# fmfi-compbio/nadavca

Measured on AMD Instinct MI355X. Metric: reads/sec (align_signal, ~4k-sample reads), higher is better.
Workload: dtype f64

## Files before the change

### nadavca_amd/csrc/api.hip

```cpp
#include <math.h>
#include <stdarg.h>
#include <stdio.h>
#include <stdlib.h>
#include <string.h>

#include <new>
#include <vector>

#include "nvk_internal.h"

static thread_local char g_err[512] = "";

void nvk_set_error(const char *fmt, ...) {
  va_list ap;
  va_start(ap, fmt);
  vsnprintf(g_err, sizeof g_err, fmt, ap);
  va_end(ap);
}

extern "C" const char *nvk_last_error(void) { return g_err; }

extern "C" int nvk_device_count(void) {
  int n = 0;
  if (hipGetDeviceCount(&n) != hipSuccess) return 0;
// ... 387 lines not shown
  }
  NVK_HIP(hipSetDevice(model->ctx->device));
  a = BatchArgs{n_reads, total_signal, total_ref, total_anchors, signal, sig_off, reference, ref_off,
                ctx_before, cb_off, ctx_after, ca_off, anchors, anc_off, bandwidth, mel};
  return NVK_OK;
}

struct PlanHost {
  PlanTotals tot;
  int32_t steps[1];
};

int plan_batch_queue(nvk_model *model, const BatchArgs &a, int mode, int write_rows, const int **order,
                     const std::function<int()> *meanwhile) {
  nvk_ctx *ctx = model->ctx;
  int64_t n = a.n_reads;
  int64_t rows_total = (mode == PLAN_ALIGN_TRANS) ? 2 * a.total_ref : a.total_ref + n;
  int rc;
  ctx->rows_current = 0;
  if ((rc = nvk_ws_reserve(ctx, WS_META, (size_t)(n + 1) * sizeof(ReadMeta) + 64))) return rc;
  if ((rc = nvk_ws_reserve(ctx, WS_ROWS, (size_t)(rows_total + 1) * sizeof(RowParam)))) return rc;
  if ((rc = nvk_ws_reserve(ctx, WS_BANDTMP, (size_t)(2 * (a.total_ref + n) + 2) * 8))) return rc;
  if ((rc = nvk_ws_reserve(ctx, WS_MISC, 256))) return rc;
  if ((rc = nvk_ws_reserve(ctx, WS_LANE_F, (size_t)(rows_total + 1) * 48))) return rc;
  if ((rc = nvk_ws_reserve(ctx, WS_LANE_R, (size_t)(rows_total + 1) * 48))) return rc;
  if ((rc = nvk_ws_reserve(ctx, WS_OFFS, (size_t)(rows_total + 1) * sizeof(int32_t)))) return rc;
  if ((rc = nvk_ws_reserve(ctx, WS_STEPS, (size_t)(n + 1) * sizeof(int32_t)))) return rc;
  if ((rc = nvk_ws_reserve(ctx, WS_ORDER, (size_t)n * sizeof(int) + 4096))) return rc;
  if ((rc = nvk_grow(&ctx->h_plan, &ctx->h_plan_cap, sizeof(PlanHost) + (size_t)n * sizeof(int32_t), true,
                     "planner results")))
    return rc;
  PlanTotals *d_tot = nvk_plan_totals(ctx);
  rc = launch_plan(ctx, model->dm, a, mode, (ReadMeta *)ctx->ws[WS_META],
                   (RowParam *)ctx->ws[WS_ROWS], (unsigned long long *)ctx->ws[WS_BANDTMP], d_tot,
                   ctx->ws[WS_LANE_F], ctx->ws[WS_LANE_R], (int32_t *)ctx->ws[WS_OFFS], write_rows, meanwhile);
  if (rc) return rc;
  ctx->rows_current = write_rows ? 1 : 0;
  int *ord = nullptr;
  rc = launch_order(ctx, (const ReadMeta *)ctx->ws[WS_META], n, d_tot, &ord, (int32_t *)ctx->ws[WS_STEPS]);
  if (rc) return rc;
  *order = ord;
  return NVK_OK;
}

int plan_batch_wait(nvk_ctx *ctx, int64_t n, PlanTotals &tot, const int32_t **steps_sorted) {
  PlanHost *hp = (PlanHost *)ctx->h_plan;
  NVK_HIP(hipMemcpyAsync(&hp->tot, nvk_plan_totals(ctx), sizeof(PlanTotals), hipMemcpyDeviceToHost, ctx->stream));
  if (n) NVK_HIP(hipMemcpyAsync(hp->steps, ctx->ws[WS_STEPS], (size_t)n * sizeof(int32_t), hipMemcpyDeviceToHost,
// ... 299 lines not shown
```

### nadavca_amd/csrc/kernels_align.hip

```cpp
#include <math.h>

#include "nvk_internal.h"
#include "wave.h"
#include "xmath.h"

namespace {

using xm::X;

constexpr int CH = 128;
constexpr int TABN = 128;
constexpr int PF = 4;

struct AlignArgs {
  const ReadMeta *metas;
  const RowParam *rows;
  const double *signal;
  double *spill_m;
  int32_t *spill_e;
  uint32_t *bp;
  int64_t spill_stride;
  int64_t bp_stride;
  int n_reads;
  int *counter;
// ... 327 lines not shown
            e = density(ring[(i - 1) & RM], mean, ac2, mc2);
            su = (su + 1 == H) ? 0 : su + 1;
            sA = (sA + 1 == H) ? 0 : sA + 1;
            sB = (sB + 1 == H) ? 0 : sB + 1;
            WAVE_SYNC();
          }
        }
#pragma unroll
        for (int q = 0; q < PF; q++) {
          cur_m[q] = nxt_m[q];
          cur_e[q] = nxt_e[q];
        }
      }
    }
    __syncthreads();

    int idx = __shfl(fidx, top & 63, 64);
    if (idx < 0) {
      if (lane == 0) g.out_status[rd] = NVK_READ_NO_PATH;
      continue;
    }
    {
      const bool ax = __any(amb_x), an = __any(amb_n), au = __any(amb_u);
      if ((ax || an || au || m.rsv) && lane == 0)
        g.ties[rd] = (ax ? NVK_TIE_EXACT : 0) | (an ? NVK_TIE_NEAR : 0) | (au ? NVK_TIE_ULP : 0) |
                     (m.rsv ? NVK_TIE_PLATEAU : 0);
    }
    if (lane == 0) {
      int32_t *ev = g.out_events + 2 * m.ref_off;
      int st = NVK_READ_OK;
      for (int r = top; r >= 0; --r) {
        if (g.transitions) {
          ev[2 * (r >> 1) + (r & 1)] = idx;
        } else {
          if (r > 0) ev[2 * (r - 1) + 1] = idx;
          if (r < top) ev[2 * r] = idx;
        }
        if (r == 0) break;
        const int pm = g.transitions ? ((r - 1) & 1 ? 0 : MEL) : MEL;
        int u = idx + c * r - t_min;
        int w = u >> 5;
        uint32_t v = bp[(size_t)w * 64 + (r & 63)] & (0xffffffffu >> (31 - (u & 31)));
        while (v == 0 && w > 0) {
          --w;
          v = bp[(size_t)w * 64 + (r & 63)];
        }
        if (v == 0) {
          st = NVK_READ_NO_PATH;
          break;
// ... 120 lines not shown
```

### nadavca_amd/csrc/kernels_align3.hip

```cpp
#include <math.h>

#include <new>
#include <vector>

#include "nvk_internal.h"
#include "xmath.h"
#include "dens.h"
#include "lane3.h"
#include "wave.h"

namespace {

using dens::density;
using dens::density_begin;
using dens::density_end;
using dens::DensHalf;
using dens::ETN;

constexpr int CH = 64;
static_assert(CH == 64, "a refill is one sample per lane");
constexpr int PF = 8;
constexpr int RU = 16;
constexpr int FT = 16;
static_assert(FT % PF == 0 && 32 % FT == 0, "forward trip");
// ... 9 lines not shown
typedef int v4i_t __attribute__((ext_vector_type(4)));
__device__ __forceinline__ void spill_store2(__amdgpu_buffer_rsrc_t rs, int lane16, int pair, double v_even,
                                             double v_odd) {
  __builtin_amdgcn_raw_buffer_store_b128(__builtin_bit_cast(v4i_t, make_double2(v_even, v_odd)), rs, lane16,
                                         pair * 1024, SPILL_AUX);
}
__device__ __forceinline__ double2 spill_load2(__amdgpu_buffer_rsrc_t rs, int lane16, int pair) {
  return __builtin_bit_cast(double2, __builtin_amdgcn_raw_buffer_load_b128(rs, lane16, pair * 1024, SPILL_AUX));
}

#define STEP_SYNC()                                                              \
  do {                                                                           \
    if (W == 1) WAVE_SYNC();                                                     \
    else asm volatile("s_waitcnt lgkmcnt(0)\n\ts_barrier" ::: "memory");         \
  } while (0)
#define RING_SYNC()                 \
  do {                              \
    if (W == 1) __syncthreads();    \
    else WAVE_SYNC();               \
  } while (0)

struct Align3Args {
  const ReadMeta *metas;
  const Lane3 *fwdl;
  const Lane3 *revl;
  const int32_t *offs;
  const double *signal;
  double *spill_v;
  int32_t *spill_L;
  uint32_t *bp;
  int64_t spill_stride;
  int64_t L_stride;
  int64_t bp_stride;
  int n_reads;
  int *counter;
  const int *order;
  int H, SR;
  int transitions;
  int c_cap;
  int flag_above;
  int2 *rstate;
  int read_lo;
  int *n_retry;
  int32_t *ties;
  int32_t *out_events;
  int32_t *out_status;
};

#define TAKE_LANE(l)                                                                   \
  do {                                                                                 \
    if (!PAIR || em) { mean = (l).mean; ac2 = (l).ac; mc2 = (l).mc; }   \
    melr = (l).mg & 15;                                                                \
    D = ((l).mg >> 4) & 255;                                                           \
    bs = (l).bs; pA = (l).pA; pW = (l).pW;                                             \
    ra = (int)min((unsigned)(su - D), (unsigned)(su - D + H)) * TL + nb;               \
    if (!PAIR) { pm = melr ? 1.0 : 0.0; qm = melr ? 0.0 : 1.0; }                       \
    if (PAIR && !em) cq = (shift_now != 0) ? ldexp((l).mean, shift_now) : (l).mean;    \
  } while (0)

__device__ __forceinline__ Lane3 lane3_sload(const Lane3 *p) {
  typedef const __attribute__((address_space(4))) v4i_t *cptr_t;
  cptr_t q = (cptr_t)(uintptr_t)p;
  const v4i_t q0 = q[0], q1 = q[1], q2 = q[2];
  Lane3 l;
  l.mean = __hiloint2double(q0.y, q0.x);
  l.ac = __hiloint2double(q0.w, q0.z);
  l.mc = __hiloint2double(q1.y, q1.x);
  l.bs = q1.z; l.end = q1.w;
  l.lo = q2.x; l.pA = q2.y; l.pW = q2.z; l.mg = q2.w;
  return l;
}

__device__ __forceinline__ int pair_swap(int v) { return __builtin_amdgcn_mov_dpp(v, 0xB1, 0xf, 0xf, true); }
__device__ __forceinline__ double pair_swap(double v) {
  return __hiloint2double(pair_swap(__double2hiint(v)), pair_swap(__double2loint(v)));
}

template <int MEL>
__device__ __forceinline__ double emission_product(double e, double e1, double e2, double e3) {
  double P = 1.0;
  if (MEL >= 1) P = e;
  if (MEL >= 2) P = P * e1;
  if (MEL >= 3) P = P * e2;
  if (MEL >= 4) P = P * e3;
  return P;
}

__device__ __forceinline__ int wave_max_i(int v) {
  for (int d = 32; d >= 1; d >>= 1) v = max(v, __shfl_xor(v, d, 64));
  return __builtin_amdgcn_readfirstlane(v);
}

struct Scale {
// ... 37 lines not shown
    }
  }
  unsigned char *histb = reinterpret_cast<unsigned char *>(hist2);
  unsigned char *ghistb = reinterpret_cast<unsigned char *>(ghist);
  int gl16 = gl * 16, gl8 = gl * 8, HZv = HZ, HZ2v = (PHASE == 1) ? HZ : 2 * HZ;
  asm volatile("" : "+v"(gl16), "+v"(gl8), "+v"(HZv), "+v"(HZ2v));
  const int lane16 = (W == 1) ? gl16 : lane * 16;

  while (true) {
    __syncthreads();
    if (gl == 0) *s_read = atomicAdd(g.counter, 1);
    __syncthreads();
    const int pos0 = __builtin_amdgcn_readfirstlane(*s_read);
    if (pos0 >= g.n_reads) break;
    const int pos = pos0 + g.read_lo;
    const int rd = g.order ? g.order[pos] : pos;
    const ReadMeta m = g.metas[rd];
    if (m.status != NVK_READ_OK) {
      if (PHASE == 2 && gl == 0) g.out_status[rd] = m.status;
      continue;
    }
    if ((W > 1) != (m.cw != 0)) continue;
    const int cm = (W > 1) ? m.cw : m.c;
    if (cm > g.c_cap) {
      if (PHASE == 2 && g.flag_above && gl == 0) {
        g.out_status[rd] = NVK_READ_RETRY_INTERNAL;
        atomicAdd(g.n_retry, 1);
      }
      continue;
    }
    const size_t slot = (size_t)pos0;
    const __amdgpu_buffer_rsrc_t spill_rs = __builtin_amdgcn_make_buffer_rsrc(
        g.spill_v + (slot * W + wv) * g.spill_stride, 0, 0x7ffffff0, 0x00020000);
    int32_t *spill_L = g.spill_L + slot * g.L_stride;
    const int T = __builtin_amdgcn_readfirstlane(m.T);
    const int N = __builtin_amdgcn_readfirstlane(m.N);
    const int c = __builtin_amdgcn_readfirstlane(cm);
    const int t_min = __builtin_amdgcn_readfirstlane(m.t_min);
    const int n_steps = __builtin_amdgcn_readfirstlane(m.pad);
    const int t_max = t_min + n_steps - 1;
    const Lane3 *fwdl = g.fwdl + m.row_off;
    const Lane3 *revl = g.revl + m.row_off;
    const int32_t *offs = g.offs + m.row_off;
    const double *sig = g.signal + m.sig_off;
    const int top = T - 1;
    int K = 0;
    bool suspect = false;

    if (PHASE == 1) {
      int r = top - ((top - gl) & (TL - 1));
      double mean = 0, ac2 = 0, mc2 = 0;
      int bs = -0x40000000, hi = -0x40000000, pA = 0x40000000, pW = 0, melr = 0, D = 1;
      double pm = 0.0, qm = 1.0;
      const bool em = PAIR ? ((lane & 1) == 0) : true;
      double cq = 0.0;
      int ia = 0;
      int dsel = 0;
      int shift_now = 0;
      if (PAIR) { pm = em ? 1.0 : 0.0; qm = em ? 0.0 : 1.0; }
      int su = 0;
      const int nb = (gl + 1) & (TL - 1);
      int ra = (H - 1) * TL + nb;
      bool is_init = false;
      int i = t_max;
      if (r >= 0) {
        const Lane3 cu = revl[r];
        TAKE_LANE(cu);
        hi = cu.end;
        is_init = (r == top);
        i = t_max - offs[r];
      }
      double prev = 0.0, e1 = 1.0, e2 = 1.0, e3 = 1.0;
      double o_hold = 0.0;
      int kmax = -0x40000000;
      int r_old = (W == 1) ? top : max(wave_max_i(r), -1);
      int i_old = (r_old >= 0) ? __builtin_amdgcn_readlane(i, r_old & 63) : 0x40000000;
      int filled_lo = (i_old / CH + 1) * CH;
      while (i_old - 3 < filled_lo) {
        filled_lo -= CH;
        for (int q = lane; q < CH; q += 64) {
          int idx = filled_lo + q;
          ring[idx & RM] = (idx >= 0 && idx < N) ? sig[idx] : 0.0;
        }
      }
      double nxt;
      {
        const int idx = filled_lo - CH + lane;
        nxt = (idx >= 0 && idx < N) ? sig[idx] : 0.0;
      }
// ... 16 lines not shown
      for (int ub = 0; ub < n_steps; ub += RU) {
#pragma unroll
      for (int uq = 0; uq < RU; uq++) {
        const int u = ub + uq;
        const int t = t_max - u;
        const int age = u & (RS - 1);
        if (age == 0 && u > 0) {
          sc.L += sc.d_next;
          sc.d_last = sc.d_next;
          sh_until = (sc.d_next != 0) ? u + c + MEL : 0;
          sc.d_next = 0;
          if (PAIR) { cq = ldexp(cq, sc.d_last); dsel = 0; }
        }
        if (PAIR && age == 1 && u > 1) cq = ldexp(cq, -sc.d_last);
        shift_now = (age == 0 && u > 0) ? sc.d_last : 0;
        bool fin = (i < bs);
        if (__any(fin)) {
          bool redo = false;
          for (unsigned long long fm = __builtin_amdgcn_ballot_w64(fin); fm != 0; fm &= fm - 1) {
            const int fl = __builtin_ctzll(fm);
            const int rn = __builtin_amdgcn_readlane(r, fl) - TL;
            Lane3 nx;
            nx.mean = nx.ac = nx.mc = 0.0; nx.bs = nx.end = nx.lo = nx.pA = nx.pW = nx.mg = 0;
            if (rn >= 0) nx = lane3_sload(revl + rn);
            if (lane == fl) {
              r = rn;
              i += nx.mg >> 12;
              prev = 0.0;
              if (r >= 0) {
                TAKE_LANE(nx);
                hi = nx.end;
                is_init = false;
                redo = true;
              } else {
                hi = -0x40000000; bs = -0x40000000; pA = 0x40000000; pW = 0;
                if (PAIR && !em) cq = 0.0;
              }
            }
          }
          if (PAIR) {
            if (__any(redo && em)) {
              const double pmn = pair_swap(mean), pac = pair_swap(ac2), pmc = pair_swap(mc2);
              const int ip = pair_swap(i);
              if (!em) { mean = pmn; ac2 = pac; mc2 = pmc; }
              const int odd = u & 1;
              if (W > 1) {
                redo = em ? redo : !odd;
// ... 118 lines not shown
      suspect = (rs.y != 0);
    }
    __syncthreads();
    __builtin_amdgcn_s_dcache_inv();

    double fbest = 0.0, fthr = 0.0;
    int fidx = -1, fG = 0;
    unsigned long long amb_x = 0, amb_u = 0, amb_n = 0;
    {
      int r = gl;
      double mean = 0, ac2 = 0, mc2 = 0;
      int bs = 0, be = 0x40000000, lo = 0x40000000, pA = 0x40000000, pW = 0, melr = 0, D = 1;
      double pm = 0.0, qm = 1.0;
      const bool em = PAIR ? ((lane & 1) != 0) : true;
      double cq = 0.0;
      int ia = 0, dsel = 0, shift_now = 0;
      if (PAIR) { pm = em ? 1.0 : 0.0; qm = em ? 0.0 : 1.0; }
      int su = 0;
      const int nb = (gl - 1) & (TL - 1);
      int ra = (H - 1) * TL + nb;
      bool is_init = false;
      int i = t_min - 64 * c;
      if (r < T) {
        const Lane3 cu = fwdl[r];
        TAKE_LANE(cu);
        be = cu.end; lo = cu.lo;
        is_init = (r == 0);
        i = t_min - offs[r];
      }
      double prev = 0.0, e1 = 1.0, e2 = 1.0, e3 = 1.0;
      double bestn = 0.0, bthr = 0.0;
      int G = GBIG;
      double rsum = 0.0, smin = INFINITY, smax = 0.0;
      uint32_t bits = 0;
      int r_old = min(64 * wv, T);
      int i_old = (r_old < T) ? __builtin_amdgcn_readfirstlane(i) : -0x40000000;
      int filled_hi = ((i_old - MEL - 1) > 0 ? (i_old - MEL - 1) / CH : 0) * CH;
      while (i_old + 2 >= filled_hi) {
        for (int w = lane; w < CH; w += 64) {
          int idx = filled_hi + w;
          ring[idx & RM] = (idx >= 0 && idx < N) ? sig[idx] : 0.0;
        }
        filled_hi += CH;
      }
      double nxt;
      {
        const int idx = filled_hi + lane;
// ... 25 lines not shown
      for (int ub = 0; ub < n_steps; ub += FT) {
#pragma unroll
        for (int q = 0; q < FT; q++) {
          const int u = ub + q;
          {
            const int age = u & (RS - 1);
            if (age == 0 && u > 0) {
              sc.L += sc.d_next;
              sc.d_last = sc.d_next;
              sh_until = (sc.d_next != 0) ? u + c + MEL : 0;
              sc.d_next = 0;
              if (PAIR) { cq = ldexp(cq, sc.d_last); dsel = 0; }
            }
            if (PAIR && age == 1 && u > 1) cq = ldexp(cq, -sc.d_last);
            shift_now = (age == 0 && u > 0) ? sc.d_last : 0;
            bool fin = (i > be);
            if (__any(fin)) {
              bool redo = false;
              for (unsigned long long fm = __builtin_amdgcn_ballot_w64(fin); fm != 0; fm &= fm - 1) {
                const int fl = __builtin_ctzll(fm);
                const int rn = __builtin_amdgcn_readlane(r, fl) + TL;
                Lane3 nx;
                nx.mean = nx.ac = nx.mc = 0.0; nx.bs = nx.end = nx.lo = nx.pA = nx.pW = nx.mg = 0;
                if (rn < T) nx = lane3_sload(fwdl + rn);
                if (lane == fl) {
                  smin = fmin(smin, rsum);
                  smax = fmax(smax, rsum);
                  rsum = 0.0;
                  r = rn;
                  i -= nx.mg >> 12;
                  prev = 0.0;
                  bestn = 0.0; bthr = 0.0; G = GBIG;
                  if (r < T) {
                    TAKE_LANE(nx);
                    be = nx.end; lo = nx.lo;
                    is_init = false;
                    redo = true;
                  } else {
                    lo = 0x40000000; be = 0x40000000; pA = 0x40000000; pW = 0;
                    if (PAIR && !em) cq = 0.0;
                  }
                }
              }
              if (PAIR) {
                if (__any(redo && em)) {
                  const double pmn = pair_swap(mean), pac = pair_swap(ac2), pmc = pair_swap(mc2);
                  const int ip = pair_swap(i);
// ... 169 lines not shown
      if (lane == 0) tflag[wv] = (any_suspect ? 1 : 0) | (amb_x != 0 ? 2 : 0) | (amb_n != 0 ? 4 : 0) | (amb_u != 0 ? 8 : 0);
      if (gl == (top & (TL - 1))) *tfidx = fidx;
      __syncthreads();
      int fl = 0;
#pragma unroll
      for (int w = 0; w < W; w++) fl |= tflag[w];
      any_suspect = (fl & 1) != 0;
      amb_x = (fl & 2) ? 1ull : 0ull;
      amb_n = (fl & 4) ? 1ull : 0ull;
      amb_u = (fl & 8) ? 1ull : 0ull;
      idx = *tfidx;
    }
    if (any_suspect || (idx < 0 && K != 0)) {
      if (gl == 0) {
        g.out_status[rd] = NVK_READ_RETRY_INTERNAL;
        atomicAdd(g.n_retry, 1);
      }
      continue;
    }
    if (idx < 0) {
      if (gl == 0) g.out_status[rd] = NVK_READ_NO_PATH;
      continue;
    }
    if (gl == 0 && ((amb_x | amb_n | amb_u) != 0 || m.rsv))
      g.ties[rd] = (amb_x != 0 ? NVK_TIE_EXACT : 0) | (amb_n != 0 ? NVK_TIE_NEAR : 0) | (amb_u != 0 ? NVK_TIE_ULP : 0) |
                   (m.rsv ? NVK_TIE_PLATEAU : 0);
    if (wv == 0) {
      int32_t *ev = g.out_events + 2 * m.ref_off;
      const float steps_per_row = (float)n_steps / (float)T;
      int st = NVK_READ_OK;
      int r = top;
      int cur = __builtin_amdgcn_readfirstlane(idx);
      while (r >= 0) {
        const int r0 = r;
        const int l = lane >> 2, q = lane & 3;
        const int row = r0 - l;
        const int off_l = (row >= 0) ? offs[row] : 0;
        const int pm_l = g.transitions ? ((row - 1) & 1 ? 0 : MEL) : MEL;
        const int a_l = off_l - t_min;
        const int b_l = t_min - off_l - pm_l;
        const int u0 = cur + __builtin_amdgcn_readfirstlane(a_l);
        const int wq = ((u0 - (int)((float)l * steps_per_row)) >> 5) + 1 - q;
        const uint32_t word = (row >= 1 && wq >= 0) ? bp[(size_t)wq * TL + (row & (TL - 1))] : 0u;
        int curs = cur;
        int done = 0;
        for (int ll = 0; ll < 16; ++ll) {
          curs = (lane == ll) ? cur : curs;
          done = ll + 1;
          if (r == 0) {
// ... 135 lines not shown
      nvk_set_error("no align3 kernel for min_event_length %d, transitions %d, %d waves, rescale period %d", mel,
                    transitions, W, 1 << rsh);
      return NVK_ERR_UNSUPPORTED;
    }
    const int H = (c + mel > 0 ? c + mel : 1) + (W > 1 ? 1 : 0);
    int SR = 256;
    while (SR < 64 * c + CH) SR <<= 1;
    const size_t lds = lds_need(c, 20);
    const size_t lds_rev = lds_need(c, 8);
    if (lds > 160 * 1024) return NVK_ERR_UNSUPPORTED;
    int per_cu = (int)((160 * 1024) / lds);
    if (per_cu > 4 * LB / W) per_cu = 4 * LB / W;
    if (per_cu < 1) per_cu = 1;
    int per_cu_rev = (int)((160 * 1024) / lds_rev);
    if (per_cu_rev > 4 * (W > 1 ? LB_REV_TEAM : LB_REV) / W) per_cu_rev = 4 * (W > 1 ? LB_REV_TEAM : LB_REV) / W;
    if (per_cu_rev < 1) per_cu_rev = 1;
    int32_t mxpad = 1;
    for (int64_t q = 0; q < a.n_reads; q++) mxpad = steps_sorted[q] > mxpad ? steps_sorted[q] : mxpad;
    const int64_t bp_stride = (int64_t)((mxpad + 31) / 32 + 1) * TLk;
    const int64_t cap = (k == 0) ? spill_cap : nvk_spill_cap(ctx, WS_SPILL);

    Align3Args g;
    g.metas = metas;
    g.fwdl = (const Lane3 *)ctx->ws[WS_LANE_F];
    g.revl = (const Lane3 *)ctx->ws[WS_LANE_R];
    g.offs = (const int32_t *)ctx->ws[WS_OFFS];
    g.signal = a.signal;
    g.bp_stride = bp_stride;
    g.order = order;
    g.H = H;
    g.SR = SR;
    g.transitions = transitions;
    g.c_cap = c;
    g.flag_above = (k == ncls - 1) ? 1 : 0;
    g.rstate = (int2 *)ctx->ws[WS_RSTATE];
    g.n_retry = d_retry;
    g.ties = (int32_t *)ctx->ws[WS_TIES];
    g.out_events = out_events;
    g.out_status = out_status;
    for (int ph = 0; ph < 2; ph++)
      if ((ph == 0 ? lds_rev : lds) > 64 * 1024)
        NVK_HIP(hipFuncSetAttribute((const void *)kern[ph], hipFuncAttributeMaxDynamicSharedMemorySize,
                                    (int)(ph == 0 ? lds_rev : lds)));
    const int64_t pos_lo = (W > 1) ? 0 : n_wide, pos_hi = (W > 1) ? n_wide : a.n_reads;
    int64_t lo = pos_lo;
    while (lo < pos_hi) {
      int64_t hi = lo, mx = 1;
      while (hi < pos_hi) {
// ... 47 lines not shown
```

### nadavca_amd/csrc/kernels_plan.hip

```cpp
#include <math.h>

#include "nvk_internal.h"
#include "kmer.h"
#include "lane3.h"
#include "wave.h"

namespace {

__device__ __forceinline__ int read_is_bad(const DeviceModel &dm, const BatchArgs &a, int rd, int tid,
                                           int nthreads) {
  const int64_t s0 = a.sig_off[rd], s1 = a.sig_off[rd + 1], r0 = a.ref_off[rd], r1 = a.ref_off[rd + 1];
  const int64_t a0 = a.anc_off[rd], a1 = a.anc_off[rd + 1];
  const int64_t b0 = a.cb_off[rd], b1 = a.cb_off[rd + 1], c0 = a.ca_off[rd], c1 = a.ca_off[rd + 1];
  const int64_t N64 = s1 - s0, R64 = r1 - r0;
  if (s0 < 0 || r0 < 0 || a0 < 0 || b0 < 0 || c0 < 0 || a1 < a0 || b1 < b0 || c1 < c0 ||
      s1 > a.total_signal || r1 > a.total_ref || a1 > a.total_anchors || b1 - b0 > 0x3fffffff ||
      c1 - c0 > 0x3fffffff)
    return 1;
  if (R64 < 1 || N64 < 1 || N64 > 0x3fffffff || R64 > 0x1fffffff) return 1;
  const int R = (int)R64, A = (int)(a1 - a0), nb = (int)(b1 - b0), na = (int)(c1 - c0);
  const int32_t *anc = a.anchors + 2 * a0;
  const int32_t *ref = a.reference + r0, *cb = a.ctx_before + b0, *ca = a.ctx_after + c0;
  int bad = 0;
  for (int j = tid; j < A && !bad; j += nthreads) {
// ... 52 lines not shown
      if (j <= R) {
        unsigned long long w = tbe[j];
        v = (w >> 32) ? (int)(unsigned int)(w & 0xffffffffu) - 1 : N;
      } else {
        v = 0x7fffffff;
      }
      v = min(wave_scan_min_dpp(v), carry);
      carry = __builtin_amdgcn_readlane(v, 63);
      if (j <= R) be[j] = (W)(unsigned int)v;
    }
  }
  __syncthreads();
}

constexpr int PLAN_T = 256;
constexpr int PLAN_VT = 2048;
constexpr int PLAN_BCAP = 1024;

struct PlanShared {
  unsigned long long pool[3 * PLAN_VT / 2];
  unsigned int ids[PLAN_BCAP];
  unsigned long long cells;
  int c, cw, var;
};
static_assert(2 * PLAN_BCAP * 8 <= 2 * PLAN_VT * 4 && 2 * PLAN_BCAP <= PLAN_VT, "LDS layout of PlanStoreLds");

struct PlanRead {
  const int32_t *ref, *cb, *ca, *anc;
  int64_t r0;
  int N, R, A, T, nb, na, bw, mel;
};

struct PlanStoreLds {
  PlanShared &sh;
  __device__ __forceinline__ int *b() const { return (int *)sh.pool + 2 * PLAN_VT; }
  __device__ __forceinline__ void bands(const PlanRead &q, int tid) const {
    plan_bands(q.anc, q.A, q.R, q.N, q.bw, sh.pool, sh.pool + PLAN_BCAP, b(), b() + PLAN_BCAP, tid, PLAN_T);
  }
  __device__ __forceinline__ int bs(int j) const { return b()[j]; }
  __device__ __forceinline__ int be(int j) const { return b()[PLAN_BCAP + j]; }
  __device__ __forceinline__ void fill_ids(const DeviceModel &dm, const PlanRead &q, int first, int stride) const {
    for (int i = first; i < q.R; i += stride)
      sh.ids[i] = (unsigned int)kmer_id(dm, q.ref, q.R, q.cb, q.nb, q.ca, q.na, i);
  }
  __device__ __forceinline__ unsigned int kid(const DeviceModel &, const PlanRead &, int i) const { return sh.ids[i]; }
};
struct PlanStoreGlobal {
  unsigned long long *tbs, *tbe;
  __device__ __forceinline__ void bands(const PlanRead &q, int tid) const {
    plan_bands(q.anc, q.A, q.R, q.N, q.bw, tbs, tbe, tbs, tbe, tid, PLAN_T);
  }
  __device__ __forceinline__ int bs(int j) const { return (int)(unsigned int)tbs[j]; }
  __device__ __forceinline__ int be(int j) const { return (int)(unsigned int)tbe[j]; }
  __device__ __forceinline__ void fill_ids(const DeviceModel &, const PlanRead &, int, int) const {}
  __device__ __forceinline__ int64_t kid(const DeviceModel &dm, const PlanRead &q, int i) const {
    return kmer_id(dm, q.ref, q.R, q.cb, q.nb, q.ca, q.na, i);
  }
};

template <class Store>
__device__ __forceinline__ void plan_rows(const Store st, const DeviceModel &dm, const PlanRead &q, int mode,
                                          double log_p_in, int c_cap, int rd, ReadMeta m, ReadMeta *metas,
                                          RowParam *rows, bool write_rows, Lane3 *lane_f, Lane3 *lane_r,
                                          int32_t *lane_offs, PlanShared &sh) {
  const int tid = threadIdx.x, lane = tid & 63, wv = tid >> 6;
  const int N = q.N, T = q.T, mel = q.mel;
  const bool trans = (mode == PLAN_ALIGN_TRANS);
  constexpr int VT = PLAN_VT;
  int *sh_x = (int *)sh.pool, *sh_S = sh_x + VT;
  st.bands(q, tid);

  auto rmel = [=](int r) { return (r + 1 < T && !(trans && (r & 1))) ? mel : 0; };
  auto BS = [=](int r) { return st.bs(trans ? (r + 1) >> 1 : r); };
  auto BE = [=](int r) { return st.be(trans ? (r + 1) >> 1 : r); };
  auto LO = [=](int r) {
    int lo = BS(r);
    if (r > 0) {
      const int pm = rmel(r - 1);
      lo = min(lo, BS(r - 1) + pm) - max(pm - 1, 0);
    }
    return lo;
  };
  auto HI = [=](int r) {
    int hi = BE(r);
    if (r + 1 < T) {
      const int pm = rmel(r);
// ... 25 lines not shown
  }
  __syncthreads();
  const int c = sh.c;
  const bool team = (c > c_cap);
  int cw = 0;
  if (team) {
    constexpr int TL = 64 * ALIGN3_TEAM_W;
    if (tid == 0) sh.cw = max(mel - 1, 1);
    __syncthreads();
    int need = 1;
    for (int r = TL + tid; r < T; r += PLAN_T) {
      int d = HI(r - TL) - LO(r) + idle;
      if (d >= 0) need = max(need, d / TL + 1);
    }
    need = wave_max(need);
    if (lane == 0) atomicMax(&sh.cw, need);
    __syncthreads();
    cw = sh.cw;
  }

  const int gmin = max(mel - 1, 1);
  const bool neg_gaps = trans && mel <= 2;
  const bool fixp = !team && T <= VT && T > 64 && (neg_gaps || c > gmin);
  if (tid == 0) sh.var = 0;
  if (fixp) {
    for (int r = tid; r < T; r += PLAN_T) {
      int g = 0;
      if (r > 0) {
        g = gmin;
        if (neg_gaps) g = max(1 - rmel(r - 1), max(LO(r - 1) - LO(r), HI(r - 1) - HI(r)));
        g = min(g, c);
      }
      sh_S[r] = g;
      sh_x[r] = 0;
    }
  }
  __syncthreads();
  const int t0 = fixp ? 64 : 0;
  if (tid >= t0) st.fill_ids(dm, q, tid - t0, PLAN_T - t0);
  {
    if (fixp && tid < 64) {
      int carry = 0;
      for (int b0 = 0; b0 < T; b0 += 64) {
        const int r = b0 + lane;
        const int v = wave_scan_add_dpp(r < T ? sh_S[r] : 0) + carry;
        if (r < T) sh_S[r] = v;
        carry = __builtin_amdgcn_readlane(v, 63);
// ... 49 lines not shown
          if (r < T) {
            const int nx = z + U;
            changed |= (nx != cur);
            sh_x[r] = nx;
          }
          carryz = __builtin_amdgcn_readlane(z, 63);
        }
        WAVE_SYNC();
        changed = __any(changed);
      }
      if (lane == 0) sh.var = changed ? 0 : 1;
    }
    __syncthreads();
  }
  const bool var_ok = (sh.var != 0);
  const int x0 = var_ok ? sh_x[0] : 0;
  const int cu = team ? cw : c;
  auto OFF = [=](int r) { return var_ok ? sh_x[r] - x0 + sh_S[r] : cu * r; };

  RowParam *rp = rows + m.row_off;
  const bool records = lane_f && !badband;
  const int top = T - 1;
  const int ST = cw ? 64 * ALIGN3_TEAM_W : 64;
  int plateau = 0;
  for (int base = 0; base < T; base += 63 * (PLAN_T / 64)) {
    const int r = base + 63 * wv + lane - 1;
    const bool have = (r >= 0 && r < T);
    RowParam o;
    o.mean = 0.0;
    o.ac = 0.0;
    o.mc = 0.0;
    o.mel = 0;
    o.bs = o.be = o.lo = o.hi = o.off = 0;
    if (have && r + 1 < T) {
      if (trans && (r & 1)) {
        int i = r / 2;
        double m1 = dm.mean[st.kid(dm, q, i)];
        double m2 = dm.mean[st.kid(dm, q, i + 1)];
        o.ac = (m1 == m2) ? -INFINITY : log_p_in;
        plateau |= (m1 == m2) ? 1 : 0;
      } else {
        int i = trans ? r / 2 : r;
        const auto id = st.kid(dm, q, i);
        o.mean = dm.mean[id];
        o.ac = dm.ac[id];
        o.mc = dm.mc[id];
        o.mel = mel;
      }
    }
    RowParam p, nx;
// ... 5 lines not shown
    nx.bs = nx.be = nx.lo = nx.hi = nx.mel = nx.off = 0;
    if (have && lane > 0) {
      o.bs = BS(r);
      o.be = BE(r);
      o.lo = LO(r);
      o.hi = HI(r);
      o.off = OFF(r);
      if (!trans && r > 0 && r + 1 < T) plateau |= (p.mean == o.mean) ? 1 : 0;
      if (write_rows) rp[r] = o;
      if (records) {
        if (r > 0) {
          p.bs = BS(r - 1);
          p.be = BE(r - 1);
          p.mel = rmel(r - 1);
          p.off = OFF(r - 1);
        }
        if (r < top) {
          nx.bs = BS(r + 1);
          nx.be = BE(r + 1);
          nx.off = OFF(r + 1);
        }
        const int adv_f = (r >= ST) ? o.off - OFF(r - ST) : 0;
        const int adv_b = (r + ST <= top) ? OFF(r + ST) - o.off : 0;
        Lane3 f, b;
        lane3_row(o, p, r > 0, nx, r < top, N, adv_f, adv_b, f, b);
        (lane_f + m.row_off)[r] = f;
        (lane_r + m.row_off)[r] = b;
        (lane_offs + m.row_off)[r] = o.off;
      }
    }
  }
  plateau = __syncthreads_or(plateau);

  if (tid == 0) {
    const int hi_top = HI(T - 1);
    int t_min = LO(0);
    int t_max = hi_top + c * (T - 1);
    m.c = c;
    m.cw = cw;
    m.t_min = t_min;
    m.n_steps = t_max - t_min + 1;
    m.pad = hi_top + OFF(T - 1) - t_min + 1;
    m.pad = (m.pad + 31) & ~31;
    m.cells = (long long)sh.cells;
    m.rsv = plateau ? 1 : 0;
    if (badband) m.status = NVK_READ_BAD_BAND;
    metas[rd] = m;
  }
}

__global__ __launch_bounds__(PLAN_T, 5) void plan_kernel(DeviceModel dm, BatchArgs a, int mode,
                                                  double log_p_in, int c_cap, ReadMeta *metas,
                                                  RowParam *rows, unsigned long long *bandtmp,
                                                  Lane3 *lane_f, Lane3 *lane_r, int32_t *lane_offs, int write_rows) {
  const int rd = blockIdx.x;
  const int tid = threadIdx.x;
  __shared__ PlanShared sh;
  if (rd >= a.n_reads) return;
  if (tid == 0) {
    sh.cells = 0ull;
    sh.c = 1;
  }
  const int64_t s0 = a.sig_off[rd], r0 = a.ref_off[rd], a0 = a.anc_off[rd];
  const int64_t N64 = a.sig_off[rd + 1] - s0;
  const int64_t R64 = a.ref_off[rd + 1] - r0;
  const int64_t A64 = a.anc_off[rd + 1] - a0;
  PlanRead q;
  q.nb = (int)(a.cb_off[rd + 1] - a.cb_off[rd]);
  q.na = (int)(a.ca_off[rd + 1] - a.ca_off[rd]);
  q.ref = a.reference + r0;
  q.cb = a.ctx_before + a.cb_off[rd];
  q.ca = a.ctx_after + a.ca_off[rd];
  q.anc = a.anchors + 2 * a0;
  q.r0 = r0;
  q.N = (int)N64;
  q.R = (int)R64;
  q.A = (int)A64;
// ... 304 lines not shown
  NVK_HIP(hipMemsetAsync(cnt, 0, 2 * ORD_N * sizeof(int), ctx->stream));
  const unsigned blocks = (unsigned)((n_reads + 255) / 256);
  TimerScope ts(ctx, NVK_K_PLAN);
  hipLaunchKernelGGL(order_count_kernel, dim3(blocks), dim3(256), 0, ctx->stream, metas, (int)n_reads, tot_dev, cnt);
  hipLaunchKernelGGL(order_scan_kernel, dim3(1), dim3(64), 0, ctx->stream, cnt);
  hipLaunchKernelGGL(order_fill_kernel, dim3(blocks), dim3(256), 0, ctx->stream, metas, (int)n_reads, tot_dev, cnt, ord,
                     steps_out);
  NVK_HIP(hipGetLastError());
  *order = ord;
  return NVK_OK;
}

int launch_plan(nvk_ctx *ctx, const DeviceModel &dm, const BatchArgs &a, int mode,
                ReadMeta *metas, RowParam *rows, unsigned long long *bandtmp, PlanTotals *totals,
                void *lane_f, void *lane_r, int32_t *lane_offs, int write_rows,
                const std::function<int()> *meanwhile) {
  if (totals) NVK_HIP(hipMemsetAsync(totals, 0, sizeof(PlanTotals), ctx->stream));
  if (a.n_reads == 0) return meanwhile ? (*meanwhile)() : NVK_OK;
  int rc = NVK_OK;
  {
    TimerScope ts(ctx, NVK_K_PLAN);
    const double log_p_in = log(0.01);
    hipLaunchKernelGGL(plan_kernel, dim3((unsigned)a.n_reads), dim3(PLAN_T), 0, ctx->stream, dm, a, mode,
                       log_p_in, ALIGN1_C_CAP, metas, rows, bandtmp, (Lane3 *)lane_f, (Lane3 *)lane_r, lane_offs,
                       write_rows);
    if (totals)
      hipLaunchKernelGGL(plan_totals_kernel, dim3((unsigned)((a.n_reads + 255) / 256)), dim3(256), 0, ctx->stream,
                         metas, (int)a.n_reads, ALIGN1_C_CAP, totals);
    ts.stop();
    if (meanwhile) rc = (*meanwhile)();
  }
  NVK_HIP(hipGetLastError());
  return rc;
}

int launch_plan_ell(nvk_ctx *ctx, const DeviceModel &dm, const BatchArgs &a, int wobbling,
                    const EllPlan &pl, unsigned long long *bandtmp, PlanTotals *totals) {
  NVK_HIP(hipMemsetAsync(totals, 0, sizeof(PlanTotals), ctx->stream));
  if (a.n_reads == 0) return NVK_OK;
  {
    TimerScope ts(ctx, NVK_K_PLAN);
    hipLaunchKernelGGL(plan_ell_kernel, dim3((unsigned)a.n_reads), dim3(64), 0, ctx->stream, dm, a,
                       wobbling, pl, bandtmp, totals);
  }
  NVK_HIP(hipGetLastError());
  return NVK_OK;
}
// ... 15 lines not shown
```

### nadavca_amd/csrc/lane3.h

```cpp
#pragma once
#include "nvk_internal.h"
#include "dens.h"

struct __attribute__((aligned(16))) Lane3 {
  double mean, ac, mc;
  int32_t bs;
  int32_t end;
  int32_t lo;
  int32_t pA, pW;
  int32_t mg;
};
__device__ __forceinline__ int lane3_pack(int mel, int age, int adv) { return mel | (age << 4) | (adv * 4096); }
static_assert(sizeof(Lane3) == 48, "Lane3 layout");

__device__ __forceinline__ void set_density_consts(Lane3 &l, const RowParam &o) {
  l.mean = o.mean;
  dens::scale_consts(o.ac, o.mc, l.ac, l.mc);
  if (l.mc == 0.0) l.mean = dens::constant_density(l.ac);
}


__device__ __forceinline__ void lane3_row(const RowParam &o, const RowParam &p, bool has_p, const RowParam &q,
                                          bool has_q, int N, int adv_f, int adv_b, Lane3 &f, Lane3 &b) {
  f.bs = o.bs; f.end = o.be; f.lo = o.lo;
  if (has_p) {
    set_density_consts(f, p);
    f.lo = max(o.lo, p.mel);
    {
      const int a = max(f.lo, p.bs + p.mel), z = min(o.be, p.be + p.mel);
      f.pA = (z >= a) ? a : 0x40000000; f.pW = (z >= a) ? z - a : 0;
    }
    f.mg = lane3_pack(p.mel, o.off - p.off + p.mel, adv_f);
  } else {
    f.mean = 1.0; f.ac = 0.0; f.mc = 0.0; f.mg = lane3_pack(0, 1, 0); f.pA = 0x40000000; f.pW = 0;
  }
  set_density_consts(b, o);
  b.bs = o.bs; b.lo = 0;
  if (has_q) {
    b.end = min(o.hi, N - o.mel);
    {
      const int a = max(o.bs, q.bs - o.mel), z = min(b.end, q.be - o.mel);
      b.pA = (z >= a) ? a : 0x40000000; b.pW = (z >= a) ? z - a : 0;
    }
    b.mg = lane3_pack(o.mel, q.off - o.off + o.mel, adv_b);
  } else {
    b.pA = 0x40000000; b.pW = 0;
    b.end = o.hi;
    b.mg = lane3_pack(o.mel, 1 + o.mel, adv_b);
  }
}
```

Baseline: 712,800.

## Pack reverse lane records into 64-byte row pairs for transition alignment

In transitions mode, reverse-pass lane records are stored as 64-byte pairs: shared density constants, a second mean for odd rows, and two 16-byte packed integer blocks with 16-bit deltas. This replaces two 48-byte Lane3 records per pair, cutting scalar and vector load traffic in the backward pass, and the planner writes rows in 62-row strides so a pair never crosses waves. Reads whose fields overflow the packing are marked with a new rsv bit and routed to retry, and the plateau check now masks rsv to bit 0. The cost is extra unpack arithmetic per row load and a new fallback path.

```diff
diff --git a/nadavca_amd/csrc/api.hip b/nadavca_amd/csrc/api.hip
--- a/nadavca_amd/csrc/api.hip
+++ b/nadavca_amd/csrc/api.hip
@@ -433,8 +433,10 @@
   if ((rc = nvk_ws_reserve(ctx, WS_ROWS, (size_t)(rows_total + 1) * sizeof(RowParam)))) return rc;
   if ((rc = nvk_ws_reserve(ctx, WS_BANDTMP, (size_t)(2 * (a.total_ref + n) + 2) * 8))) return rc;
   if ((rc = nvk_ws_reserve(ctx, WS_MISC, 256))) return rc;
-  if ((rc = nvk_ws_reserve(ctx, WS_LANE_F, (size_t)(rows_total + 1) * 48))) return rc;
-  if ((rc = nvk_ws_reserve(ctx, WS_LANE_R, (size_t)(rows_total + 1) * 48))) return rc;
+  const size_t lane3_bytes = (size_t)(rows_total + 1) * 48;
+  if ((rc = nvk_ws_reserve(ctx, WS_LANE_F, lane3_bytes))) return rc;
+  if ((rc = nvk_ws_reserve(ctx, WS_LANE_R, (mode == PLAN_ALIGN_TRANS) ? (size_t)(rows_total + 2) * 32 : lane3_bytes)))
+    return rc;
   if ((rc = nvk_ws_reserve(ctx, WS_OFFS, (size_t)(rows_total + 1) * sizeof(int32_t)))) return rc;
   if ((rc = nvk_ws_reserve(ctx, WS_STEPS, (size_t)(n + 1) * sizeof(int32_t)))) return rc;
   if ((rc = nvk_ws_reserve(ctx, WS_ORDER, (size_t)n * sizeof(int) + 4096))) return rc;
diff --git a/nadavca_amd/csrc/kernels_align.hip b/nadavca_amd/csrc/kernels_align.hip
--- a/nadavca_amd/csrc/kernels_align.hip
+++ b/nadavca_amd/csrc/kernels_align.hip
@@ -373,9 +373,9 @@
     }
     {
       const bool ax = __any(amb_x), an = __any(amb_n), au = __any(amb_u);
-      if ((ax || an || au || m.rsv) && lane == 0)
+      if ((ax || an || au || (m.rsv & 1)) && lane == 0)
         g.ties[rd] = (ax ? NVK_TIE_EXACT : 0) | (an ? NVK_TIE_NEAR : 0) | (au ? NVK_TIE_ULP : 0) |
-                     (m.rsv ? NVK_TIE_PLATEAU : 0);
+                     ((m.rsv & 1) ? NVK_TIE_PLATEAU : 0);
     }
     if (lane == 0) {
       int32_t *ev = g.out_events + 2 * m.ref_off;
diff --git a/nadavca_amd/csrc/kernels_align3.hip b/nadavca_amd/csrc/kernels_align3.hip
--- a/nadavca_amd/csrc/kernels_align3.hip
+++ b/nadavca_amd/csrc/kernels_align3.hip
@@ -55,8 +55,8 @@
 
 struct Align3Args {
   const ReadMeta *metas;
-  const Lane3 *fwdl;
-  const Lane3 *revl;
+  const void *fwdl;
+  const void *revl;
   const int32_t *offs;
   const double *signal;
   double *spill_v;
@@ -91,17 +91,50 @@
     if (PAIR && !em) cq = (shift_now != 0) ? ldexp((l).mean, shift_now) : (l).mean;    \
   } while (0)
 
-__device__ __forceinline__ Lane3 lane3_sload(const Lane3 *p) {
+typedef int v8i_t __attribute__((ext_vector_type(8)));
+__device__ __forceinline__ void lane3_ints(Lane3 &l, const v4i_t w) {
+  const LaneInts v = lane_unpack(w.x, w.y, w.z, w.w);
+  l.bs = v.bs; l.end = v.end; l.lo = v.lo; l.pA = v.pA; l.pW = v.pW; l.mg = v.mg;
+}
+template <bool PAIR>
+__device__ __forceinline__ Lane3 lane3_sload(const unsigned char *recs, int row, bool emits) {
   typedef const __attribute__((address_space(4))) v4i_t *cptr_t;
-  cptr_t q = (cptr_t)(uintptr_t)p;
-  const v4i_t q0 = q[0], q1 = q[1], q2 = q[2];
+  typedef const __attribute__((address_space(4))) v8i_t *cptr8_t;
   Lane3 l;
-  l.mean = __hiloint2double(q0.y, q0.x);
-  l.ac = __hiloint2double(q0.w, q0.z);
-  l.mc = __hiloint2double(q1.y, q1.x);
-  l.bs = q1.z; l.end = q1.w;
-  l.lo = q2.x; l.pA = q2.y; l.pW = q2.z; l.mg = q2.w;
+  if constexpr (PAIR) {
+    const uintptr_t rec = (uintptr_t)recs + (size_t)(row >> 1) * sizeof(LanePair);
+    const v8i_t q = *(cptr8_t)rec;
+    const v4i_t w = *(cptr_t)(rec + offsetof(LanePair, blk) + 16 * (row & 1));
+    int t0 = q[6], t1 = q[7];
+    asm("" : "+s"(t0), "+s"(t1));
+    l.mean = emits ? __hiloint2double(q[1], q[0]) : __hiloint2double(t1, t0);
+    l.ac = __hiloint2double(q[3], q[2]);
+    l.mc = __hiloint2double(q[5], q[4]);
+    lane3_ints(l, w);
+  } else {
+    cptr_t q = (cptr_t)((uintptr_t)recs + (size_t)row * sizeof(Lane3));
+    const v4i_t q0 = q[0], q1 = q[1], q2 = q[2];
+    l.mean = __hiloint2double(q0.y, q0.x);
+    l.ac = __hiloint2double(q0.w, q0.z);
+    l.mc = __hiloint2double(q1.y, q1.x);
+    l.bs = q1.z; l.end = q1.w;
+    l.lo = q2.x; l.pA = q2.y; l.pW = q2.z; l.mg = q2.w;
+  }
   return l;
+}
+template <bool PAIR>
+__device__ __forceinline__ Lane3 lane3_vload(const unsigned char *recs, int row, bool emits) {
+  if constexpr (PAIR) {
+    const LanePair *rec = reinterpret_cast<const LanePair *>(recs) + (row >> 1);
+    Lane3 l;
+    l.mean = emits ? rec->mean : rec->tconst;
+    l.ac = rec->ac;
+    l.mc = rec->mc;
+    lane3_ints(l, *reinterpret_cast<const v4i_t *>(rec->blk[row & 1]));
+    return l;
+  } else {
+    return reinterpret_cast<const Lane3 *>(recs)[row];
+  }
 }
 
 __device__ __forceinline__ int pair_swap(int v) { return __builtin_amdgcn_mov_dpp(v, 0xB1, 0xf, 0xf, true); }
@@ -185,8 +218,9 @@
     }
     if ((W > 1) != (m.cw != 0)) continue;
     const int cm = (W > 1) ? m.cw : m.c;
-    if (cm > g.c_cap) {
-      if (PHASE == 2 && g.flag_above && gl == 0) {
+    const bool nofit = PAIR && (m.rsv & 2);
+    if (cm > g.c_cap || nofit) {
+      if (PHASE == 2 && (g.flag_above || nofit) && gl == 0) {
         g.out_status[rd] = NVK_READ_RETRY_INTERNAL;
         atomicAdd(g.n_retry, 1);
       }
@@ -202,8 +236,9 @@
     const int t_min = __builtin_amdgcn_readfirstlane(m.t_min);
     const int n_steps = __builtin_amdgcn_readfirstlane(m.pad);
     const int t_max = t_min + n_steps - 1;
-    const Lane3 *fwdl = g.fwdl + m.row_off;
-    const Lane3 *revl = g.revl + m.row_off;
+    const unsigned char *fwdl = (const unsigned char *)g.fwdl + (size_t)m.row_off * sizeof(Lane3);
+    const unsigned char *revl =
+        (const unsigned char *)g.revl + (size_t)m.row_off * (PAIR ? sizeof(LanePair) / 2 : sizeof(Lane3));
     const int32_t *offs = g.offs + m.row_off;
     const double *sig = g.signal + m.sig_off;
     const int top = T - 1;
@@ -227,7 +262,7 @@
       bool is_init = false;
       int i = t_max;
       if (r >= 0) {
-        const Lane3 cu = revl[r];
+        const Lane3 cu = lane3_vload<PAIR>(revl, r, em);
         TAKE_LANE(cu);
         hi = cu.end;
         is_init = (r == top);
@@ -290,7 +325,7 @@
             const int rn = __builtin_amdgcn_readlane(r, fl) - TL;
             Lane3 nx;
             nx.mean = nx.ac = nx.mc = 0.0; nx.bs = nx.end = nx.lo = nx.pA = nx.pW = nx.mg = 0;
-            if (rn >= 0) nx = lane3_sload(revl + rn);
+            if (rn >= 0) nx = lane3_sload<PAIR>(revl, rn, (rn & 1) == 0);
             if (lane == fl) {
               r = rn;
               i += nx.mg >> 12;
@@ -455,7 +490,7 @@
       bool is_init = false;
       int i = t_min - 64 * c;
       if (r < T) {
-        const Lane3 cu = fwdl[r];
+        const Lane3 cu = lane3_vload<false>(fwdl, r, true);
         TAKE_LANE(cu);
         be = cu.end; lo = cu.lo;
         is_init = (r == 0);
@@ -527,7 +562,7 @@
                 const int rn = __builtin_amdgcn_readlane(r, fl) + TL;
                 Lane3 nx;
                 nx.mean = nx.ac = nx.mc = 0.0; nx.bs = nx.end = nx.lo = nx.pA = nx.pW = nx.mg = 0;
-                if (rn < T) nx = lane3_sload(fwdl + rn);
+                if (rn < T) nx = lane3_sload<false>(fwdl, rn, true);
                 if (lane == fl) {
                   smin = fmin(smin, rsum);
                   smax = fmax(smax, rsum);
@@ -743,9 +778,9 @@
       if (gl == 0) g.out_status[rd] = NVK_READ_NO_PATH;
       continue;
     }
-    if (gl == 0 && ((amb_x | amb_n | amb_u) != 0 || m.rsv))
+    if (gl == 0 && ((amb_x | amb_n | amb_u) != 0 || (m.rsv & 1)))
       g.ties[rd] = (amb_x != 0 ? NVK_TIE_EXACT : 0) | (amb_n != 0 ? NVK_TIE_NEAR : 0) | (amb_u != 0 ? NVK_TIE_ULP : 0) |
-                   (m.rsv ? NVK_TIE_PLATEAU : 0);
+                   ((m.rsv & 1) ? NVK_TIE_PLATEAU : 0);
     if (wv == 0) {
       int32_t *ev = g.out_events + 2 * m.ref_off;
       const float steps_per_row = (float)n_steps / (float)T;
@@ -927,8 +962,8 @@
 
     Align3Args g;
     g.metas = metas;
-    g.fwdl = (const Lane3 *)ctx->ws[WS_LANE_F];
-    g.revl = (const Lane3 *)ctx->ws[WS_LANE_R];
+    g.fwdl = ctx->ws[WS_LANE_F];
+    g.revl = ctx->ws[WS_LANE_R];
     g.offs = (const int32_t *)ctx->ws[WS_OFFS];
     g.signal = a.signal;
     g.bp_stride = bp_stride;
diff --git a/nadavca_amd/csrc/kernels_plan.hip b/nadavca_amd/csrc/kernels_plan.hip
--- a/nadavca_amd/csrc/kernels_plan.hip
+++ b/nadavca_amd/csrc/kernels_plan.hip
@@ -98,6 +98,7 @@
   unsigned int ids[PLAN_BCAP];
   unsigned long long cells;
   int c, cw, var;
+  int nofit;
 };
 static_assert(2 * PLAN_BCAP * 8 <= 2 * PLAN_VT * 4 && 2 * PLAN_BCAP <= PLAN_VT, "LDS layout of PlanStoreLds");
 
@@ -137,7 +138,7 @@
 template <class Store>
 __device__ __forceinline__ void plan_rows(const Store st, const DeviceModel &dm, const PlanRead &q, int mode,
                                           double log_p_in, int c_cap, int rd, ReadMeta m, ReadMeta *metas,
-                                          RowParam *rows, bool write_rows, Lane3 *lane_f, Lane3 *lane_r,
+                                          RowParam *rows, bool write_rows, void *lane_f, void *lane_r,
                                           int32_t *lane_offs, PlanShared &sh) {
   const int tid = threadIdx.x, lane = tid & 63, wv = tid >> 6;
   const int N = q.N, T = q.T, mel = q.mel;
@@ -209,7 +210,7 @@
   const int gmin = max(mel - 1, 1);
   const bool neg_gaps = trans && mel <= 2;
   const bool fixp = !team && T <= VT && T > 64 && (neg_gaps || c > gmin);
-  if (tid == 0) sh.var = 0;
+  if (tid == 0) sh.var = 0, sh.nofit = 0;
   if (fixp) {
     for (int r = tid; r < T; r += PLAN_T) {
       int g = 0;
@@ -305,10 +306,11 @@
   const bool records = lane_f && !badband;
   const int top = T - 1;
   const int ST = cw ? 64 * ALIGN3_TEAM_W : 64;
+  const int RW = trans ? 62 : 63;
   int plateau = 0;
-  for (int base = 0; base < T; base += 63 * (PLAN_T / 64)) {
-    const int r = base + 63 * wv + lane - 1;
-    const bool have = (r >= 0 && r < T);
+  for (int base = 0; base < T; base += RW * (PLAN_T / 64)) {
+    const int r = base + RW * wv + lane - 1;
+    const bool have = (r >= 0 && r < T && lane <= RW);
     RowParam o;
     o.mean = 0.0;
     o.ac = 0.0;
@@ -360,10 +362,21 @@
         }
         const int adv_f = (r >= ST) ? o.off - OFF(r - ST) : 0;
         const int adv_b = (r + ST <= top) ? OFF(r + ST) - o.off : 0;
+        LaneFields fb;
         Lane3 f, b;
-        lane3_row(o, p, r > 0, nx, r < top, N, adv_f, adv_b, f, b);
-        (lane_f + m.row_off)[r] = f;
-        (lane_r + m.row_off)[r] = b;
+        lane3_row(o, p, r > 0, nx, r < top, N, adv_f, adv_b, f, b, fb);
+        ((Lane3 *)lane_f + m.row_off)[r] = f;
+        if (trans) {
+          const int odd = r & 1;
+          char *pr = (char *)lane_r + (size_t)(m.row_off + r - odd) * (sizeof(LanePair) / 2);
+          int32_t w[4];
+          if (!lane_pack(fb, w)) sh.nofit = 1;
+          if (!odd) *(double2 *)(pr + offsetof(LanePair, mean)) = make_double2(b.mean, b.ac);
+          *(double *)(pr + (odd ? offsetof(LanePair, tconst) : offsetof(LanePair, mc))) = odd ? b.mean : b.mc;
+          *(int4 *)(pr + offsetof(LanePair, blk) + 16 * odd) = make_int4(w[0], w[1], w[2], w[3]);
+        } else {
+          ((Lane3 *)lane_r + m.row_off)[r] = b;
+        }
         (lane_offs + m.row_off)[r] = o.off;
       }
     }
@@ -381,7 +394,7 @@
     m.pad = hi_top + OFF(T - 1) - t_min + 1;
     m.pad = (m.pad + 31) & ~31;
     m.cells = (long long)sh.cells;
-    m.rsv = plateau ? 1 : 0;
+    m.rsv = (plateau ? 1 : 0) | (sh.nofit ? 2 : 0);
     if (badband) m.status = NVK_READ_BAD_BAND;
     metas[rd] = m;
   }
@@ -390,7 +403,7 @@
 __global__ __launch_bounds__(PLAN_T, 5) void plan_kernel(DeviceModel dm, BatchArgs a, int mode,
                                                   double log_p_in, int c_cap, ReadMeta *metas,
                                                   RowParam *rows, unsigned long long *bandtmp,
-                                                  Lane3 *lane_f, Lane3 *lane_r, int32_t *lane_offs, int write_rows) {
+                                                  void *lane_f, void *lane_r, int32_t *lane_offs, int write_rows) {
   const int rd = blockIdx.x;
   const int tid = threadIdx.x;
   __shared__ PlanShared sh;
@@ -741,7 +754,7 @@
     TimerScope ts(ctx, NVK_K_PLAN);
     const double log_p_in = log(0.01);
     hipLaunchKernelGGL(plan_kernel, dim3((unsigned)a.n_reads), dim3(PLAN_T), 0, ctx->stream, dm, a, mode,
-                       log_p_in, ALIGN1_C_CAP, metas, rows, bandtmp, (Lane3 *)lane_f, (Lane3 *)lane_r, lane_offs,
+                       log_p_in, ALIGN1_C_CAP, metas, rows, bandtmp, lane_f, lane_r, lane_offs,
                        write_rows);
     if (totals)
       hipLaunchKernelGGL(plan_totals_kernel, dim3((unsigned)((a.n_reads + 255) / 256)), dim3(256), 0, ctx->stream,
diff --git a/nadavca_amd/csrc/lane3.h b/nadavca_amd/csrc/lane3.h
--- a/nadavca_amd/csrc/lane3.h
+++ b/nadavca_amd/csrc/lane3.h
@@ -1,4 +1,62 @@
 #pragma once
+#include <stdint.h>
+
+#ifdef __HIPCC__
+#define LANE_FN __host__ __device__ __forceinline__
+#else
+#define LANE_FN inline
+#endif
+
+struct LaneFields {
+  int32_t bs, end, lo, pA, pW;
+  int32_t mel, age, adv;
+};
+struct LaneInts {
+  int32_t bs, end, lo, pA, pW, mg;
+};
+
+constexpr int32_t LANE_PA_NONE = 0x40000000;
+constexpr uint32_t LANE_W2_NONE = 0x8000u;
+
+LANE_FN int32_t lane_mg(int32_t mel, int32_t age, int32_t adv) {
+  return (int32_t)((uint32_t)mel | ((uint32_t)age << 4) | ((uint32_t)adv << 12));
+}
+
+LANE_FN bool lane_pack(const LaneFields &v, int32_t w[4]) {
+  const int64_t de = (int64_t)v.end - v.bs, dl = (int64_t)v.bs - v.lo, da = (int64_t)v.pA - v.bs;
+  bool ok = de >= -32768 && de <= 32767 && dl >= -32768 && dl <= 32767;
+  ok = ok && v.mel >= 0 && v.mel <= 15 && v.age >= 0 && v.age <= 255 && v.adv >= -(1 << 19) && v.adv < (1 << 19);
+  uint32_t w2 = LANE_W2_NONE;
+  if (!(v.pA == LANE_PA_NONE && v.pW == 0)) {
+    ok = ok && da >= -32767 && da <= 32767 && v.pW >= 0 && v.pW <= 65535;
+    w2 = ((uint32_t)da & 0xffffu) | ((uint32_t)v.pW << 16);
+  }
+  w[0] = v.bs;
+  w[1] = (int32_t)(((uint32_t)de & 0xffffu) | ((uint32_t)dl << 16));
+  w[2] = (int32_t)w2;
+  w[3] = lane_mg(v.mel, v.age, v.adv);
+  return ok;
+}
+
+LANE_FN LaneInts lane_unpack(int32_t w0, int32_t w1, int32_t w2, int32_t w3) {
+  LaneInts v;
+  v.bs = w0;
+  v.end = w0 + (int32_t)(int16_t)(uint16_t)((uint32_t)w1 & 0xffffu);
+  v.lo = w0 - (w1 >> 16);
+  v.pA = ((uint32_t)w2 == LANE_W2_NONE) ? LANE_PA_NONE : w0 + (int32_t)(int16_t)(uint16_t)((uint32_t)w2 & 0xffffu);
+  v.pW = (int32_t)((uint32_t)w2 >> 16);
+  v.mg = w3;
+  return v;
+}
+
+struct alignas(64) LanePair {
+  double mean, ac, mc;
+  double tconst;
+  int32_t blk[2][4];
+};
+static_assert(sizeof(LanePair) == 64, "LanePair layout");
+
+#ifdef __HIPCC__
 #include "nvk_internal.h"
 #include "dens.h"
 
@@ -10,7 +68,6 @@
   int32_t pA, pW;
   int32_t mg;
 };
-__device__ __forceinline__ int lane3_pack(int mel, int age, int adv) { return mel | (age << 4) | (adv * 4096); }
 static_assert(sizeof(Lane3) == 48, "Lane3 layout");
 
 __device__ __forceinline__ void set_density_consts(Lane3 &l, const RowParam &o) {
@@ -21,31 +78,36 @@
 
 
 __device__ __forceinline__ void lane3_row(const RowParam &o, const RowParam &p, bool has_p, const RowParam &q,
-                                          bool has_q, int N, int adv_f, int adv_b, Lane3 &f, Lane3 &b) {
+                                          bool has_q, int N, int adv_f, int adv_b, Lane3 &f, Lane3 &b,
+                                          LaneFields &fb) {
   f.bs = o.bs; f.end = o.be; f.lo = o.lo;
   if (has_p) {
     set_density_consts(f, p);
     f.lo = max(o.lo, p.mel);
     {
       const int a = max(f.lo, p.bs + p.mel), z = min(o.be, p.be + p.mel);
-      f.pA = (z >= a) ? a : 0x40000000; f.pW = (z >= a) ? z - a : 0;
+      f.pA = (z >= a) ? a : LANE_PA_NONE; f.pW = (z >= a) ? z - a : 0;
     }
-    f.mg = lane3_pack(p.mel, o.off - p.off + p.mel, adv_f);
+    f.mg = lane_mg(p.mel, o.off - p.off + p.mel, adv_f);
   } else {
-    f.mean = 1.0; f.ac = 0.0; f.mc = 0.0; f.mg = lane3_pack(0, 1, 0); f.pA = 0x40000000; f.pW = 0;
+    f.mean = 1.0; f.ac = 0.0; f.mc = 0.0; f.mg = lane_mg(0, 1, 0); f.pA = LANE_PA_NONE; f.pW = 0;
   }
   set_density_consts(b, o);
   b.bs = o.bs; b.lo = 0;
+  fb.mel = o.mel; fb.adv = adv_b;
   if (has_q) {
     b.end = min(o.hi, N - o.mel);
     {
       const int a = max(o.bs, q.bs - o.mel), z = min(b.end, q.be - o.mel);
-      b.pA = (z >= a) ? a : 0x40000000; b.pW = (z >= a) ? z - a : 0;
+      b.pA = (z >= a) ? a : LANE_PA_NONE; b.pW = (z >= a) ? z - a : 0;
     }
-    b.mg = lane3_pack(o.mel, q.off - o.off + o.mel, adv_b);
+    fb.age = q.off - o.off + o.mel;
   } else {
-    b.pA = 0x40000000; b.pW = 0;
+    b.pA = LANE_PA_NONE; b.pW = 0;
     b.end = o.hi;
-    b.mg = lane3_pack(o.mel, 1 + o.mel, adv_b);
+    fb.age = 1 + o.mel;
   }
+  b.mg = lane_mg(fb.mel, fb.age, fb.adv);
+  fb.bs = b.bs; fb.end = b.end; fb.lo = b.bs; fb.pA = b.pA; fb.pW = b.pW;
 }
+#endif
```

Measured after the change: 697,700. -2.1%, worse.
